# Li-Yuetao/ActiveSplat

Hardware: AMD Instinct MI355X
Metric: render+backward frames/sec at 640x480, N Gaussians (higher is better)
Workload: dtype f32; 1 GPU; BASELINE configs[2]'s render (the north star's target configuration): 2000000 Gaussians, SH degree 3, 640x480, forward (colour+radii+depth+opacity) + backward (all input gradients), frames strictly one after the other; gaussians=2000000, sh_degree=3, width=640, height=480, tile_instances_D=4842856, streams=1, parallelism=single GPU

## Files before the change

### activesplat_amd/csrc/gs_common.h

```cpp
#pragma once
#include <hip/hip_runtime.h>
#include <stdint.h>
#include <math.h>

#include <atomic>

#include "../../include/gsplat_hip.h"

namespace gs {

constexpr int kTile = GS_TILE;
constexpr int kBlock = 256;
constexpr int kWave = 64;
constexpr int kQuad = 8;
#ifndef GS_BIN_CHUNK
#define GS_BIN_CHUNK 2048
#endif
constexpr int kBinChunk = GS_BIN_CHUNK;
constexpr int kMaxLdsTiles = 8192;
constexpr int kSortChunk = 2048;
constexpr int kSortCapMax = 16384;

struct Cam {
    int W, H, gx, gy;
// ... 290 lines not shown
                                                    uint32_t row_mask = 0xffffffffu)
{
    const int K = KC > 0 ? KC : Krt;
    const int stride = sh_row_stride(K), total = nrows * K, total4 = total >> 2;
    const float* s = src + (size_t)row0 * K;
    const float4* s4 = reinterpret_cast<const float4*>(s);
    for (int q = lane; q < total4; q += kWave) {
        int e = q << 2, r = e / K, c = e - r * K;
        const int r_last = (e + 3) / K;
        if (!(((row_mask >> r) | (row_mask >> min(r_last, 31))) & 1u)) continue;
        const float4 v = load_stream(&s4[q]);
        const float vv[4] = {v.x, v.y, v.z, v.w};
#pragma unroll
        for (int t = 0; t < 4; t++) {
            slab[r * stride + c] = vv[t];
            if (++c == K) { c = 0; ++r; }
        }
    }
    for (int e = (total4 << 2) + lane; e < total; e += kWave) {
        const int r = e / K;
        if ((row_mask >> r) & 1u) slab[r * stride + (e - r * K)] = s[e];
    }
}
__device__ __forceinline__ void sh48_half_load(float4 (&v)[6], const float* __restrict__ src, int row0, int lane)
{
    const float4* s4 = reinterpret_cast<const float4*>(src + (size_t)row0 * 48);
#pragma unroll
    for (int j = 0; j < 6; j++) v[j] = load_stream(&s4[lane + kWave * j]);
}
constexpr int kShPad4 = 52;
__device__ __forceinline__ void sh48_half_to_lds4(float* slab, const float4 (&v)[6], int lane)
{
#pragma unroll
    for (int j = 0; j < 6; j++) {
        const int q = lane + kWave * j, r = q / 12, c = q - 12 * r;
        *reinterpret_cast<float4*>(slab + r * kShPad4 + 4 * c) = v[j];
    }
}
__device__ __forceinline__ void sh48_rows_to_lds4(float* slab, const float* __restrict__ src, int row0, int nrows, int lane, uint32_t row_mask = 0xffffffffu)
{
    const float4* s4 = reinterpret_cast<const float4*>(src + (size_t)row0 * 48);
    for (int q = lane; q < nrows * 12; q += kWave) {
        const int r = q / 12, c = q - 12 * r;
        if ((row_mask >> r) & 1u) *reinterpret_cast<float4*>(slab + r * kShPad4 + 4 * c) = load_stream(&s4[q]);
    }
}
template <int KC = 0>
__device__ __forceinline__ void sh_wave_rows_from_lds(const float* slab, float* __restrict__ dst, int row0, int nrows, int Krt, int lane)
{
    const int K = KC > 0 ? KC : Krt;
    const int stride = sh_row_stride(K), total = nrows * K, total4 = total >> 2;
    float* d = dst + (size_t)row0 * K;
    float4* d4 = reinterpret_cast<float4*>(d);
    for (int q = lane; q < total4; q += kWave) {
        int e = q << 2, r = e / K, c = e - r * K;
        float vv[4];
#pragma unroll
        for (int t = 0; t < 4; t++) {
            vv[t] = slab[r * stride + c];
            if (++c == K) { c = 0; ++r; }
        }
        store_stream(&d4[q], make_float4(vv[0], vv[1], vv[2], vv[3]));
    }
    for (int e = (total4 << 2) + lane; e < total; e += kWave) {
        const int r = e / K;
        d[e] = slab[r * stride + (e - r * K)];
    }
// ... 16 lines not shown
            by[5] = c21 * z; bz[5] = c21 * y;
            bx[6] = c22 * (-2.f * x); by[6] = c22 * (-2.f * y); bz[6] = c22 * (4.f * z);
            bx[7] = c23 * z; bz[7] = c23 * x;
            bx[8] = c24 * (2.f * x); by[8] = c24 * (-2.f * y);
            if (deg > 2) {
                const float c30 = -0.5900435899266435f, c31 = 2.890611442640554f, c32 = -0.4570457994644658f,
                            c33 = 0.3731763325901154f, c34 = -0.4570457994644658f, c35 = 1.445305721320277f,
                            c36 = -0.5900435899266435f;
                b[9] = c30 * y * (3.f * xx - yy); b[10] = c31 * x * y * z; b[11] = c32 * y * (4.f * zz - xx - yy);
                b[12] = c33 * z * (2.f * zz - 3.f * xx - 3.f * yy); b[13] = c34 * x * (4.f * zz - xx - yy);
                b[14] = c35 * z * (xx - yy); b[15] = c36 * x * (xx - 3.f * yy);
                bx[9] = c30 * (6.f * x * y); by[9] = c30 * (3.f * xx - 3.f * yy);
                bx[10] = c31 * y * z; by[10] = c31 * x * z; bz[10] = c31 * x * y;
                bx[11] = c32 * (-2.f * x * y); by[11] = c32 * (4.f * zz - xx - 3.f * yy); bz[11] = c32 * (8.f * y * z);
                bx[12] = c33 * (-6.f * x * z); by[12] = c33 * (-6.f * y * z); bz[12] = c33 * (6.f * zz - 3.f * xx - 3.f * yy);
                bx[13] = c34 * (4.f * zz - 3.f * xx - yy); by[13] = c34 * (-2.f * x * y); bz[13] = c34 * (8.f * x * z);
                bx[14] = c35 * (2.f * x * z); by[14] = c35 * (-2.f * y * z); bz[14] = c35 * (xx - yy);
                bx[15] = c36 * (3.f * xx - 3.f * yy); by[15] = c36 * (-6.f * x * y);
            }
        }
    }
}


#define GS_SHJ(k, gx, gy, gz)                                                                                                  \
    do {                                                                                                                        \
        const float c0_ = sh[3 * (k)], c1_ = sh[3 * (k) + 1], c2_ = sh[3 * (k) + 2];                                            \
        const float gx_ = (gx), gy_ = (gy), gz_ = (gz);                                                                         \
        J[0] = fmaf(c0_, gx_, J[0]); J[1] = fmaf(c0_, gy_, J[1]); J[2] = fmaf(c0_, gz_, J[2]);                                  \
        J[3] = fmaf(c1_, gx_, J[3]); J[4] = fmaf(c1_, gy_, J[4]); J[5] = fmaf(c1_, gz_, J[5]);                                  \
        J[6] = fmaf(c2_, gx_, J[6]); J[7] = fmaf(c2_, gy_, J[7]); J[8] = fmaf(c2_, gz_, J[8]);                                  \
    } while (0)
__device__ __forceinline__ void sh_direction_jacobian(int deg, float x, float y, float z, const float* sh, float (&J)[9])
{
#pragma unroll
    for (int q = 0; q < 9; q++) J[q] = 0.0f;
    if (deg < 1) return;
    const float C1 = 0.4886025119029199f;
    GS_SHJ(1, 0.f, -C1, 0.f); GS_SHJ(2, 0.f, 0.f, C1); GS_SHJ(3, -C1, 0.f, 0.f);
    if (deg < 2) return;
    const float c20 = 1.0925484305920792f, c21 = -1.0925484305920792f, c22 = 0.31539156525252005f, c23 = -1.0925484305920792f,
                c24 = 0.5462742152960396f;
    GS_SHJ(4, c20 * y, c20 * x, 0.f);
    GS_SHJ(5, 0.f, c21 * z, c21 * y);
    GS_SHJ(6, c22 * (-2.f * x), c22 * (-2.f * y), c22 * (4.f * z));
    GS_SHJ(7, c23 * z, 0.f, c23 * x);
// ... 35 lines not shown
{
    const double bc1 = 1.0 - pow(beta1, (double)step), bc2 = 1.0 - pow(beta2, (double)step);
    AdamCoef c;
    c.one_m_b1 = (float)(1.0 - beta1); c.b2 = (float)beta2; c.one_m_b2 = (float)(1.0 - beta2);
    c.step_size = (float)(lr / bc1); c.inv_bc2s = (float)(1.0 / sqrt(bc2)); c.eps = (float)eps;
    return c;
}

#define GS_SHC(j, k)                                                                                                           \
    do {                                                                                                                        \
        acc[0] = fmaf(b[k], f[3 * (j)], acc[0]); acc[1] = fmaf(b[k], f[3 * (j) + 1], acc[1]); acc[2] = fmaf(b[k], f[3 * (j) + 2], acc[2]);    \
    } while (0)
#define GS_SHJ4(j, gx, gy, gz)                                                                                                 \
    do {                                                                                                                        \
        const float c0_ = f[3 * (j)], c1_ = f[3 * (j) + 1], c2_ = f[3 * (j) + 2];                                               \
        const float gx_ = (gx), gy_ = (gy), gz_ = (gz);                                                                         \
        J[0] = fmaf(c0_, gx_, J[0]); J[1] = fmaf(c0_, gy_, J[1]); J[2] = fmaf(c0_, gz_, J[2]);                                  \
        J[3] = fmaf(c1_, gx_, J[3]); J[4] = fmaf(c1_, gy_, J[4]); J[5] = fmaf(c1_, gz_, J[5]);                                  \
        J[6] = fmaf(c2_, gx_, J[6]); J[7] = fmaf(c2_, gy_, J[7]); J[8] = fmaf(c2_, gz_, J[8]);                                  \
    } while (0)
#define GS_SHLOAD(g)                                                                                                           \
    const float4 q0_##g = row4[3 * (g)], q1_##g = row4[3 * (g) + 1], q2_##g = row4[3 * (g) + 2];                              \
    const float f[12] = {q0_##g.x, q0_##g.y, q0_##g.z, q0_##g.w, q1_##g.x, q1_##g.y, q1_##g.z, q1_##g.w, q2_##g.x, q2_##g.y, q2_##g.z, q2_##g.w}
__device__ __forceinline__ void sh48_color_and_jacobian(int deg, float x, float y, float z, const float (&b)[16], const float* row, bool want_j,
                                                        float (&acc)[3], float (&J)[9])
{
    const float4* row4 = reinterpret_cast<const float4*>(row);
#pragma unroll
    for (int q = 0; q < 9; q++) J[q] = 0.0f;
    acc[0] = acc[1] = acc[2] = 0.0f;
    const float C1 = 0.4886025119029199f;
    const float c20 = 1.0925484305920792f, c21 = -1.0925484305920792f, c22 = 0.31539156525252005f, c23 = -1.0925484305920792f,
                c24 = 0.5462742152960396f;
    const float c30 = -0.5900435899266435f, c31 = 2.890611442640554f, c32 = -0.4570457994644658f, c33 = 0.3731763325901154f,
                c34 = -0.4570457994644658f, c35 = 1.445305721320277f, c36 = -0.5900435899266435f;
    const float xx = x * x, yy = y * y, zz = z * z;
    {
        GS_SHLOAD(0);
        GS_SHC(0, 0);
        if (deg < 1) return;
        GS_SHC(1, 1); GS_SHC(2, 2); GS_SHC(3, 3);
        if (want_j) { GS_SHJ4(1, 0.f, -C1, 0.f); GS_SHJ4(2, 0.f, 0.f, C1); GS_SHJ4(3, -C1, 0.f, 0.f); }
    }
    if (deg < 2) return;
    {
        GS_SHLOAD(1);
        GS_SHC(0, 4); GS_SHC(1, 5); GS_SHC(2, 6); GS_SHC(3, 7);
        if (want_j) {
            GS_SHJ4(0, c20 * y, c20 * x, 0.f);
            GS_SHJ4(1, 0.f, c21 * z, c21 * y);
            GS_SHJ4(2, c22 * (-2.f * x), c22 * (-2.f * y), c22 * (4.f * z));
            GS_SHJ4(3, c23 * z, 0.f, c23 * x);
        }
    }
    {
        GS_SHLOAD(2);
        GS_SHC(0, 8);
        if (want_j) GS_SHJ4(0, c24 * (2.f * x), c24 * (-2.f * y), 0.f);
        if (deg >= 3) {
            GS_SHC(1, 9); GS_SHC(2, 10); GS_SHC(3, 11);
            if (want_j) {
                GS_SHJ4(1, c30 * (6.f * x * y), c30 * (3.f * xx - 3.f * yy), 0.f);
                GS_SHJ4(2, c31 * y * z, c31 * x * z, c31 * x * y);
                GS_SHJ4(3, c32 * (-2.f * x * y), c32 * (4.f * zz - xx - 3.f * yy), c32 * (8.f * y * z));
            }
        }
    }
    if (deg < 3) return;
    {
        GS_SHLOAD(3);
        GS_SHC(0, 12); GS_SHC(1, 13); GS_SHC(2, 14); GS_SHC(3, 15);
        if (want_j) {
            GS_SHJ4(0, c33 * (-6.f * x * z), c33 * (-6.f * y * z), c33 * (6.f * zz - 3.f * xx - 3.f * yy));
            GS_SHJ4(1, c34 * (4.f * zz - 3.f * xx - yy), c34 * (-2.f * x * y), c34 * (8.f * x * z));
            GS_SHJ4(2, c35 * (2.f * x * z), c35 * (-2.f * y * z), c35 * (xx - yy));
            GS_SHJ4(3, c36 * (3.f * xx - 3.f * yy), c36 * (-6.f * x * y), 0.f);
        }
    }
}
#undef GS_SHC
#undef GS_SHJ4
#undef GS_SHLOAD

constexpr int kShJacFloats = 10;
__device__ __forceinline__ void store_sh_jac(float2* base, size_t i, const float (&J)[9], uint32_t clamp_bits)
{
    float2* o = base + i * (kShJacFloats / 2);
    o[0] = make_float2(J[0], J[1]); o[1] = make_float2(J[2], J[3]); o[2] = make_float2(J[4], J[5]); o[3] = make_float2(J[6], J[7]);
    o[4] = make_float2(J[8], __uint_as_float(clamp_bits));
}
__device__ __forceinline__ void load_sh_jac(const float2* base, size_t i, float (&J)[9], uint32_t& clamp_bits)
{
    const float2* o = base + i * (kShJacFloats / 2);
    const float2 a = o[0], b = o[1], c = o[2], d = o[3], e = o[4];
    J[0] = a.x; J[1] = a.y; J[2] = b.x; J[3] = b.y; J[4] = c.x; J[5] = c.y; J[6] = d.x; J[7] = d.y; J[8] = e.x;
    clamp_bits = __float_as_uint(e.y);
}

hipError_t launch_preprocess_forward(const Cam& cam, int P, const float* means3D, const float* shs,
// ... 148 lines not shown
```

### activesplat_amd/csrc/preprocess.hip

```cpp
#include "gs_common.h"
#include <type_traits>

#pragma clang fp contract(off)

namespace gs {

__device__ __forceinline__ int clamp_tile(float v, int hi)
{
    v = fminf(fmaxf(v, -1048576.0f), 1048576.0f);
    int i = (int)v;
    return min(hi, max(0, i));
}

__device__ __forceinline__ void sh_basis(int deg, float x, float y, float z, float* b)
{
    b[0] = 0.28209479177387814f;
    if (deg > 0) {
        b[1] = -0.4886025119029199f * y; b[2] = 0.4886025119029199f * z; b[3] = -0.4886025119029199f * x;
        if (deg > 1) {
            const float xx = x * x, yy = y * y, zz = z * z, xy = x * y, yz = y * z, xz = x * z;
            b[4] = 1.0925484305920792f * xy;
            b[5] = -1.0925484305920792f * yz;
            b[6] = 0.31539156525252005f * (2.0f * zz - xx - yy);
            b[7] = -1.0925484305920792f * xz;
// ... 250 lines not shown
        __syncthreads();
    }
    int radius = 0;
    const uint32_t ntiles = project_gaussian<HAS_SH>(cam, P, view, i, io, tid, s_mean, s_scale, s_rot, s_cov, s_col, cov3Dp != nullptr, o_in,
                                                     sh_rgb, sh_clamp, radii, gp, ACT ? &radius : nullptr, in_band);
    if (ACT && i < P) {
        if (gp.vis_max) gp.vis_max[i] = fmaxf(gp.vis_max[i], (float)radius);
        if (gp.vis_seen) gp.vis_seen[i] = radius > 0 ? 1 : 0;
    }
    const uint32_t ws = wave_sum_u32(ntiles);
    if ((tid & 63) == 0) s_wsum[tid >> 6] = ws;
    __syncthreads();
    if (tid == 0) gp.block_sums[blockIdx.x] = s_wsum[0] + s_wsum[1] + s_wsum[2] + s_wsum[3];
}

template <bool ACT, class CamT = Cam>
__global__ __launch_bounds__(kBlock, 4) void preprocess_forward_sh48_kernel(
    typename CamArg<CamT>::type cam, int P, const float* __restrict__ means3D, const float* __restrict__ shs, const float* __restrict__ opac,
    const float* __restrict__ scales, const float* __restrict__ rots, const float* __restrict__ cov3Dp, int32_t* __restrict__ radii, GeomPtrs gp)
{
    load_device_pose(cam);
    __shared__ __attribute__((aligned(16))) float s_mean[kBlock * 3];
    __shared__ __attribute__((aligned(16))) float s_geo[kBlock * 7];
    __shared__ __attribute__((aligned(16))) float s_sh[(kBlock / kWave) * kShHalf * kShPad4];
    __shared__ uint32_t s_wsum[kBlock / kWave];
    float* const s_scale = s_geo;
    float* const s_rot = s_geo + kBlock * 3;
    float* const s_cov = s_geo;

    const int tid = threadIdx.x, lane = tid & 63, wave = tid >> 6;
    const int vbase = blockIdx.x * kBlock;
    const int view = cam.V > 1 ? (int)blockIdx.x / cam.nbv : 0;
    const int base = (cam.V > 1 ? (int)blockIdx.x - view * cam.nbv : (int)blockIdx.x) * kBlock;
    const int nrows = max(0, min(kBlock, P - base));
    if (vbase + tid < cam.gx * cam.gy) gp.tile_total[vbase + tid] = 0u;
    const int i = base + tid, io = vbase + tid;
    const int row_w = base + wave * kWave;
    const bool full = row_w + kWave <= P;
    float4 va[6];
    if (full) sh48_half_load(va, shs, row_w, lane);
    float o_in = i < P ? opac[i] : 0.0f;
    stage_rows<3>(s_mean, means3D, base, nrows, tid);
    if (cov3Dp) stage_rows<6>(s_cov, cov3Dp, base, nrows, tid);
    else {
        if (ACT && cam.act_iso) stage_rows<1>(s_scale, scales, base, nrows, tid); else stage_rows<3>(s_scale, scales, base, nrows, tid);
        stage_rows<4>(s_rot, rots, base, nrows, tid);
    }
    __syncthreads();
    if (ACT) o_in = activate_staged_rows(cam, tid, tid < nrows, s_mean, s_scale, s_rot, o_in);

    float sh_rgb[3] = {0.f, 0.f, 0.f};
    uint32_t sh_clamp = 0;
    float* slab = s_sh + wave * kShHalf * kShPad4;
    for (int h = 0; h < kWave / kShHalf; h++) {
        const int row0 = row_w + h * kShHalf;
        if (row0 >= P) break;
        __builtin_amdgcn_wave_barrier();
        if (full) {
            sh48_half_to_lds4(slab, va, lane);
            if (h == 0) sh48_half_load(va, shs, row_w + kShHalf, lane);
        } else {
            sh48_rows_to_lds4(slab, shs, row0, min(kShHalf, P - row0), lane);
        }
        __builtin_amdgcn_wave_barrier();
        if ((lane >> 5) == h && i < P) {
            const float* cp = cam.campos + 3 * view;
            const float dx = s_mean[tid * 3] - cp[0], dy = s_mean[tid * 3 + 1] - cp[1], dz = s_mean[tid * 3 + 2] - cp[2];
            const float inv = 1.0f / sqrtf((dx * dx + dy * dy) + dz * dz);
            float b[16];
            sh_basis(cam.sh_degree, dx * inv, dy * inv, dz * inv, b);
            float acc[3], J[9];
            sh48_color_and_jacobian(cam.sh_degree, dx * inv, dy * inv, dz * inv, b, slab + (lane & 31) * kShPad4, gp.sh_jac != nullptr, acc, J);
            acc[0] += 0.5f; acc[1] += 0.5f; acc[2] += 0.5f;
            sh_clamp = (acc[0] < 0.f ? 1u : 0u) | (acc[1] < 0.f ? 0x100u : 0u) | (acc[2] < 0.f ? 0x10000u : 0u);
            if (gp.sh_jac) store_sh_jac(gp.sh_jac, (size_t)io, J, sh_clamp);
                sh_rgb[0] = acc[0] < 0.f ? 0.f : acc[0]; sh_rgb[1] = acc[1] < 0.f ? 0.f : acc[1]; sh_rgb[2] = acc[2] < 0.f ? 0.f : acc[2];
        }
    }
    int radius = 0;
    const uint32_t ntiles = project_gaussian<true>(cam, P, view, i, io, tid, s_mean, s_scale, s_rot, s_cov, nullptr, cov3Dp != nullptr, o_in,
                                                   sh_rgb, sh_clamp, radii, gp, ACT ? &radius : nullptr);
    if (ACT && i < P) {
        if (gp.vis_max) gp.vis_max[i] = fmaxf(gp.vis_max[i], (float)radius);
        if (gp.vis_seen) gp.vis_seen[i] = radius > 0 ? 1 : 0;
    }
    const uint32_t ws = wave_sum_u32(ntiles);
    if (lane == 0) s_wsum[wave] = ws;
    __syncthreads();
    if (tid == 0) gp.block_sums[blockIdx.x] = s_wsum[0] + s_wsum[1] + s_wsum[2] + s_wsum[3];
}

__global__ __launch_bounds__(1024) void scan_block_sums_kernel(uint32_t* __restrict__ block_sums, int n, uint32_t* __restrict__ d_total)
{
    __shared__ uint32_t s_w[16];
    __shared__ uint32_t s_carry;
    const int tid = threadIdx.x, lane = tid & 63, wave = tid >> 6;
    if (tid == 0) s_carry = 0;
    __syncthreads();
    for (int base = 0; base < n; base += 1024) {
// ... 84 lines not shown
```

### activesplat_amd/csrc/preprocess_bwd.hip

```cpp
#include "gs_common.h"

namespace gs {

#ifndef GS_PBWD_RAW_SH_WGS
#define GS_PBWD_RAW_SH_WGS 4
#endif
template <bool NOALIAS> struct ParamPtr { typedef const float* __restrict__ type; };
template <> struct ParamPtr<false> { typedef const float* type; };

template <int SH, bool ACT = false, bool ADAM = false, int POSE = 0, class CamT = Cam>
__global__ __launch_bounds__(kBlock, (ACT && SH == 3) ? GS_PBWD_RAW_SH_WGS : 4) void preprocess_backward_kernel(
    typename CamArg<CamT>::type cam, int P, typename ParamPtr<!ADAM>::type means3D, typename ParamPtr<!ADAM>::type shs,
    typename ParamPtr<!ADAM>::type scales, typename ParamPtr<!ADAM>::type rots, const float* __restrict__ cov3Dp,
    const int32_t* __restrict__ radii, const uint32_t* __restrict__ clamped, const float2* __restrict__ sh_jac,
    const float* __restrict__ grad2d, float* __restrict__ dmeans2D, float* __restrict__ dmeans3D, float* __restrict__ dopac,
    float* __restrict__ dcolors, float* __restrict__ dshs, float* __restrict__ dscales,
    float* __restrict__ drots, float* __restrict__ dcov3D, typename ParamPtr<!ADAM>::type logit, FusedAdam ad, float* __restrict__ pose_rows)
{
    static_assert(POSE == 0 || (ACT && !ADAM && SH != 1), "the pose gradient is a raw-parameter mode without the optimiser step");
    load_device_pose(cam);
    float pacc[kPoseAcc];
    for (int k = 0; k < kPoseAcc; k++) pacc[k] = 0.f;
#define GS_PBWD_LEAVE do { if (POSE != 0) goto pose_reduce; return; } while (0)
    {
    constexpr bool HAS_SH = SH != 0;
    constexpr bool SLAB = SH == 1 || SH == 3;
    __shared__ __attribute__((aligned(16))) float s_sh[SLAB ? (kBlock / kWave) * kShHalf * kShPad : 1];
    const int tid = threadIdx.x;
    const int i = blockIdx.x * kBlock + tid;
    const bool in_range = i < P;
    if (ADAM && chain_failed(ad.fail)) {
        if (in_range) { dmeans2D[3 * i] = 0.f; dmeans2D[3 * i + 1] = 0.f; dmeans2D[3 * i + 2] = 0.f; }
        return;
    }
    if (!HAS_SH && !in_range) GS_PBWD_LEAVE;
    const int ic = in_range ? i : P - 1;
    const bool live = in_range && radii[ic] > 0;
    const float4* gr4 = reinterpret_cast<const float4*>(grad2d + (size_t)ic * kGradStride);
    const bool gate = ACT && !ADAM && !SLAB && cam.act_accumulate;
    float4 ga, gb, gc;
    if (gate) {
        if (!__any(live)) {
            if (in_range) { dmeans2D[3 * i] = 0.f; dmeans2D[3 * i + 1] = 0.f; dmeans2D[3 * i + 2] = 0.f; }
            GS_PBWD_LEAVE;
        }
        const float4 z4 = make_float4(0.f, 0.f, 0.f, 0.f);
        ga = z4; gb = z4; gc = z4;
        if (live) { ga = gr4[0]; gb = gr4[1]; gc = gr4[2]; }
    } else {
        ga = gr4[0]; gb = gr4[1]; gc = gr4[2];
    }
    float dmean[3] = {0.f, 0.f, 0.f};
    float o_m2d[3] = {0.f, 0.f, 0.f}, o_sc[3] = {0.f, 0.f, 0.f}, o_rot[4] = {0.f, 0.f, 0.f, 0.f};
    float o_cov[6] = {0.f, 0.f, 0.f, 0.f, 0.f, 0.f};
    float px = means3D[3 * ic], py = means3D[3 * ic + 1], pz = means3D[3 * ic + 2];
    float actR[3][3];
    if (ACT) {
        quat_to_rot(cam.act_q, actR);
        const float wx = px, wy = py, wz = pz;
        px = actR[0][0] * wx + actR[0][1] * wy + actR[0][2] * wz + cam.act_t[0];
        py = actR[1][0] * wx + actR[1][1] * wy + actR[1][2] * wz + cam.act_t[1];
        pz = actR[2][0] * wx + actR[2][1] * wy + actR[2][2] * wz + cam.act_t[2];
    }
    const float drgb[3] = {gb.z, gb.w, gc.x};
    uint32_t cl_in = 0u;
    float jac[9] = {0.f, 0.f, 0.f, 0.f, 0.f, 0.f, 0.f, 0.f, 0.f};
    if (HAS_SH && sh_jac) load_sh_jac(sh_jac, (size_t)ic, jac, cl_in);
    else if (HAS_SH) cl_in = clamped[ic];
    float sc_in[3] = {0.f, 0.f, 0.f};
    float4 rq_in = make_float4(0.f, 0.f, 0.f, 0.f), rq_raw = rq_in;
    float lg_in = 0.f;
    float cov_in[6] = {0.f, 0.f, 0.f, 0.f, 0.f, 0.f};
    if (cov3Dp) {
        for (int c = 0; c < 6; c++) cov_in[c] = cov3Dp[(size_t)ic * 6 + c];
    } else if (ACT) {
        if (cam.act_iso) { sc_in[0] = sc_in[1] = sc_in[2] = __expf(scales[ic]); }
        else { sc_in[0] = __expf(scales[3 * ic]); sc_in[1] = __expf(scales[3 * ic + 1]); sc_in[2] = __expf(scales[3 * ic + 2]); }
        rq_raw = reinterpret_cast<const float4*>(rots)[ic];
        lg_in = logit[ic];
        if (!live) {
            sc_in[0] = sc_in[1] = sc_in[2] = 0.f;
            rq_raw = make_float4(1.f, 0.f, 0.f, 0.f);
            lg_in = 0.f;
        }
        const float qr[4] = {rq_raw.x, rq_raw.y, rq_raw.z, rq_raw.w};
        float qa[4];
        activate_rotation(cam.act_q, cam.act_iso, qr, qa);
        rq_in = make_float4(qa[0], qa[1], qa[2], qa[3]);
    } else {
        sc_in[0] = scales[3 * ic]; sc_in[1] = scales[3 * ic + 1]; sc_in[2] = scales[3 * ic + 2];
        rq_in = reinterpret_cast<const float4*>(rots)[ic];
    }
    if (SLAB) {
        constexpr int KC = SH == 3 ? 48 : 0;
        const int deg = cam.sh_degree, nb = (deg + 1) * (deg + 1), M = KC ? 16 : cam.sh_coeffs, K = M * 3;
        const int stride = sh_row_stride(K);
        const int lane = tid & 63, wave = tid >> 6;
        float* slab = s_sh + wave * kShHalf * kShPad;
        for (int h = 0; h < kWave / kShHalf; h++) {
            const int row0 = blockIdx.x * kBlock + wave * kWave + h * kShHalf;
            if (row0 >= P) break;
            const int nrows = min(kShHalf, P - row0);
            __builtin_amdgcn_wave_barrier();
            const uint32_t live_rows = (uint32_t)(__ballot(live) >> (h * kShHalf));
            if (!sh_jac) sh_wave_rows_to_lds<KC>(slab, shs, row0, nrows, K, lane, live_rows);
            __builtin_amdgcn_wave_barrier();
            if ((lane >> 5) == h && in_range) {
                float* dsh = slab + (lane & 31) * stride;
                if (live) {
                    const float dx = px - cam.campos[0], dy = py - cam.campos[1], dz = pz - cam.campos[2];
                    const float inv = 1.0f / sqrtf(dx * dx + dy * dy + dz * dz);
                    const float ux = dx * inv, uy = dy * inv, uz = dz * inv;
                    float b[16], bx[16], by[16], bz[16];
                    sh_basis_and_grad(deg, ux, uy, uz, b, bx, by, bz);
                    const uint32_t cl = cl_in;
                    float du[3] = {0.f, 0.f, 0.f};
                    if (ADAM || sh_jac) {
                        const float jr[3][3] = {{jac[0], jac[1], jac[2]}, {jac[3], jac[4], jac[5]}, {jac[6], jac[7], jac[8]}};
                        for (int ch = 0; ch < 3; ch++) {
                            const float g = ((cl >> (8 * ch)) & 1u) ? 0.f : drgb[ch];
                            du[0] += g * jr[ch][0]; du[1] += g * jr[ch][1]; du[2] += g * jr[ch][2];
#pragma unroll
                            for (int k = 0; k < 16; k++)
                                if (k < M) dsh[3 * k + ch] = k < nb ? g * b[k] : 0.f;
                        }
                    } else {
                        for (int ch = 0; ch < 3; ch++) {
                            const float g = ((cl >> (8 * ch)) & 1u) ? 0.f : drgb[ch];
#pragma unroll
                            for (int k = 0; k < 16; k++) {
                                if (k < nb) {
                                    const float coef = dsh[3 * k + ch];
                                    dsh[3 * k + ch] = g * b[k];
                                    du[0] += g * coef * bx[k]; du[1] += g * coef * by[k]; du[2] += g * coef * bz[k];
                                } else if (k < M) {
                                    dsh[3 * k + ch] = 0.f;
                                }
                            }
                        }
                    }
                    const float dot = ux * du[0] + uy * du[1] + uz * du[2];
                    dmean[0] += (du[0] - ux * dot) * inv; dmean[1] += (du[1] - uy * dot) * inv; dmean[2] += (du[2] - uz * dot) * inv;
                } else {
                    for (int k = 0; k < K; k++) dsh[k] = 0.f;
                }
            }
            __builtin_amdgcn_wave_barrier();
            if (ADAM) {
                float4* p4 = reinterpret_cast<float4*>(ad.p[4] + (size_t)row0 * K);
                float4* m4 = reinterpret_cast<float4*>(ad.m[4] + (size_t)row0 * K);
                float4* v4 = reinterpret_cast<float4*>(ad.v[4] + (size_t)row0 * K);
                const int total4 = (nrows * K) >> 2;
                for (int q4 = lane; q4 < total4; q4 += kWave) {
                    float4 pp = load_stream(&p4[q4]), mm = load_stream(&m4[q4]), vv = load_stream(&v4[q4]);
                    const int e = q4 << 2, rr = e / K, cc = e - rr * K;
                    const float* gs_ = slab + rr * stride + cc;
                    adam_elem(pp.x, gs_[0], mm.x, vv.x, ad.c[4]); adam_elem(pp.y, gs_[1], mm.y, vv.y, ad.c[4]);
                    adam_elem(pp.z, gs_[2], mm.z, vv.z, ad.c[4]); adam_elem(pp.w, gs_[3], mm.w, vv.w, ad.c[4]);
                    store_stream(&p4[q4], pp); store_stream(&m4[q4], mm); store_stream(&v4[q4], vv);
                }
            } else if (POSE != 2) {
                sh_wave_rows_from_lds<KC>(slab, dshs, row0, nrows, K, lane);
            }
        }
        if (!in_range) GS_PBWD_LEAVE;
    }
    if (live) {
        const float* m = cam.view;
        const float* q = cam.proj;
        const float tx = m[0] * px + m[4] * py + m[8] * pz + m[12];
        const float ty = m[1] * px + m[5] * py + m[9] * pz + m[13];
        const float tz = m[2] * px + m[6] * py + m[10] * pz + m[14];
        const float limx = 1.3f * cam.tanfovx, limy = 1.3f * cam.tanfovy;
        const float txtz = tx / tz, tytz = ty / tz;
        const bool okx = !(txtz < -limx || txtz > limx), oky = !(tytz < -limy || tytz > limy);
        const float cx_ = fminf(limx, fmaxf(-limx, txtz)) * tz, cy_ = fminf(limy, fmaxf(-limy, tytz)) * tz;
        const float itz = 1.0f / tz, itz2 = itz * itz, itz3 = itz2 * itz;
        const float J00 = cam.fx * itz, J02 = -(cam.fx * cx_) * itz2, J11 = cam.fy * itz, J12 = -(cam.fy * cy_) * itz2;
        const float W0[3] = {m[0], m[4], m[8]}, W1[3] = {m[1], m[5], m[9]}, W2[3] = {m[2], m[6], m[10]};
        float T0[3], T1[3];
        for (int c = 0; c < 3; c++) { T0[c] = J00 * W0[c] + J02 * W2[c]; T1[c] = J11 * W1[c] + J12 * W2[c]; }
        float ST0[3], ST1[3];
        float Rm[3][3], s3[3] = {0.f, 0.f, 0.f};
        float r = 0.f, x = 0.f, y = 0.f, z = 0.f;
// ... 167 lines not shown
    if (dcolors) for (int c = 0; c < 3; c++) dcolors[3 * i + c] = live ? drgb[c] : 0.f;
    if (dscales) for (int c = 0; c < 3; c++) dscales[3 * i + c] = o_sc[c];
    if (drots) reinterpret_cast<float4*>(drots)[i] = make_float4(o_rot[0], o_rot[1], o_rot[2], o_rot[3]);
    if (dcov3D) for (int c = 0; c < 6; c++) dcov3D[6 * i + c] = o_cov[c];
    }
#undef GS_PBWD_LEAVE
    return;
pose_reduce:
    if (POSE != 0) pose_grad_block_row(pacc, pose_rows + (size_t)blockIdx.x * kPoseAcc);
}

hipError_t launch_preprocess_backward(const Cam& cam, int P, const float* means3D, const float* shs,
                                      const float* scales, const float* rots, const float* cov3Dp,
                                      const int32_t* radii, const uint32_t* clamped, const float2* sh_jac, const float* grad2d,
                                      float* dmeans2D, float* dmeans3D, float* dopac, float* dcolors, float* dshs,
                                      float* dscales, float* drots, float* dcov3D, const float* logit, const FusedAdam* adam, hipStream_t st,
                                      int pose_mode, float* pose_rows)
{
    const int nb = (P + kBlock - 1) / kBlock;
    const bool pose_only = pose_mode == 2;
    if (cam.act && (cov3Dp || !logit || !scales || !rots || (!adam && !pose_only && (!dscales || !drots)) || (shs && cam.sh_coeffs != 16))) return hipErrorInvalidValue;
    if (adam && (!cam.act || cam.act_accumulate)) return hipErrorInvalidValue;
    if (pose_mode && (!cam.act || adam || !pose_rows || pose_mode > 2)) return hipErrorInvalidValue;
    const FusedAdam ad = adam ? *adam : FusedAdam{};
#define GS_PBWD(...) hipLaunchKernelGGL((preprocess_backward_kernel<__VA_ARGS__>), dim3(nb), dim3(kBlock), 0, st, cam, P, means3D, shs, scales, rots, \
                                        cov3Dp, radii, clamped, sh_jac, grad2d, dmeans2D, dmeans3D, dopac, dcolors, dshs, dscales, drots, dcov3D, logit, ad, \
                                        pose_rows)
    if (nb > 0 && pose_mode) {
        if (shs) { if (pose_only) GS_PBWD(3, true, false, 2, Cam); else GS_PBWD(3, true, false, 1, Cam); }
        else { if (pose_only) GS_PBWD(0, true, false, 2, Cam); else GS_PBWD(0, true, false, 1, Cam); }
    }
    else if (nb > 0 && shs && cam.sh_coeffs == 16) { if (adam) GS_PBWD(3, true, true); else if (cam.act) GS_PBWD(3, true); else GS_PBWD(3, false); }
    else if (nb > 0 && shs) GS_PBWD(1, false);
    else if (nb > 0) { if (adam) GS_PBWD(0, true, true); else if (cam.act) GS_PBWD(0, true); else GS_PBWD(0, false); }
#undef GS_PBWD
    return hipGetLastError();
}

hipError_t launch_preprocess_backward_pose_dev(const CamDP& cam, int P, const float* means3D, const float* shs, const float* scales,
                                               const float* rots, const int32_t* radii, const uint32_t* clamped, const float2* sh_jac,
                                               const float* grad2d, float* dmeans2D, const float* logit, float* pose_rows, hipStream_t st)
{
    const int nb = (P + kBlock - 1) / kBlock;
    if (!cam.act || !logit || !scales || !rots || !pose_rows || (shs && cam.sh_coeffs != 16)) return hipErrorInvalidValue;
    const FusedAdam ad{};
#define GS_PBWD_DEV(SH_) hipLaunchKernelGGL((preprocess_backward_kernel<SH_, true, false, 2, CamDP>), dim3(nb), dim3(kBlock), 0, st, cam, P, means3D, \
                                            shs, scales, rots, nullptr, radii, clamped, sh_jac, grad2d, dmeans2D, nullptr, nullptr, nullptr, \
                                            nullptr, nullptr, nullptr, nullptr, logit, ad, pose_rows)
    if (nb > 0 && shs) GS_PBWD_DEV(3);
    else if (nb > 0) GS_PBWD_DEV(0);
#undef GS_PBWD_DEV
    return hipGetLastError();
}

}
```

Measured before the change: 1491 frames/s.

## Stage SH coefficients in column halves and skip backward SH re-read with saved Jacobian

The forward preprocess now stages each wave's 64 SH rows in two coefficient halves (24 floats per row, padded to 28) in LDS, so every lane handles its own Gaussian in each pass instead of half the wave idling over 32-row halves. The second half is skipped when the SH degree is below 2. In the backward, when a saved SH Jacobian is available (or Adam is fused), a new path writes dSH straight from the basis times the colour gradient in two halves. It no longer loads the SH coefficients or computes basis gradients, and takes the direction gradient from the saved Jacobian. This cuts global reads and ALU in the backward, at the cost of a new template parameter and a requirement that Adam always has sh_jac.

```diff
diff --git a/activesplat_amd/csrc/gs_common.h b/activesplat_amd/csrc/gs_common.h
--- a/activesplat_amd/csrc/gs_common.h
+++ b/activesplat_amd/csrc/gs_common.h
@@ -336,27 +336,47 @@
         if ((row_mask >> r) & 1u) slab[r * stride + (e - r * K)] = s[e];
     }
 }
-__device__ __forceinline__ void sh48_half_load(float4 (&v)[6], const float* __restrict__ src, int row0, int lane)
-{
-    const float4* s4 = reinterpret_cast<const float4*>(src + (size_t)row0 * 48);
-#pragma unroll
-    for (int j = 0; j < 6; j++) v[j] = load_stream(&s4[lane + kWave * j]);
-}
-constexpr int kShPad4 = 52;
-__device__ __forceinline__ void sh48_half_to_lds4(float* slab, const float4 (&v)[6], int lane)
-{
+constexpr int kShCoefHalf = 24;
+constexpr int kShPadC = 28;
+__device__ __forceinline__ float4 sh48_load_piece(const float4* p, bool stream)
+{
+    return stream ? load_stream(p) : *p;
+}
+__device__ __forceinline__ void sh48_chalf_load(float4 (&v)[6], const float* __restrict__ src, int row0, int half, int lane, bool stream)
+{
+    const float4* s4 = reinterpret_cast<const float4*>(src + (size_t)row0 * 48) + 6 * half;
 #pragma unroll
     for (int j = 0; j < 6; j++) {
-        const int q = lane + kWave * j, r = q / 12, c = q - 12 * r;
-        *reinterpret_cast<float4*>(slab + r * kShPad4 + 4 * c) = v[j];
-    }
-}
-__device__ __forceinline__ void sh48_rows_to_lds4(float* slab, const float* __restrict__ src, int row0, int nrows, int lane, uint32_t row_mask = 0xffffffffu)
-{
-    const float4* s4 = reinterpret_cast<const float4*>(src + (size_t)row0 * 48);
-    for (int q = lane; q < nrows * 12; q += kWave) {
-        const int r = q / 12, c = q - 12 * r;
-        if ((row_mask >> r) & 1u) *reinterpret_cast<float4*>(slab + r * kShPad4 + 4 * c) = load_stream(&s4[q]);
+        const int q = lane + kWave * j, r = q / 6, c = q - 6 * r;
+        v[j] = sh48_load_piece(&s4[12 * r + c], stream);
+    }
+}
+__device__ __forceinline__ void sh48_chalf_to_lds(float* slab, const float4 (&v)[6], int lane)
+{
+#pragma unroll
+    for (int j = 0; j < 6; j++) {
+        const int q = lane + kWave * j, r = q / 6, c = q - 6 * r;
+        *reinterpret_cast<float4*>(slab + r * kShPadC + 4 * c) = v[j];
+    }
+}
+__device__ __forceinline__ void sh48_chalf_rows_to_lds(float* slab, const float* __restrict__ src, int row0, int nrows, int half, int lane, bool stream)
+{
+    const float4* s4 = reinterpret_cast<const float4*>(src + (size_t)row0 * 48) + 6 * half;
+    for (int q = lane; q < nrows * 6; q += kWave) {
+        const int r = q / 6, c = q - 6 * r;
+        *reinterpret_cast<float4*>(slab + r * kShPadC + 4 * c) = sh48_load_piece(&s4[12 * r + c], stream);
+    }
+}
+__device__ __forceinline__ void sh48_store_piece(float4* p, const float4& x, bool stream)
+{
+    if (stream) store_stream(p, x); else *p = x;
+}
+__device__ __forceinline__ void sh48_chalf_rows_from_lds(const float* slab, float* __restrict__ dst, int row0, int nrows, int half, int lane, bool stream)
+{
+    float4* d4 = reinterpret_cast<float4*>(dst + (size_t)row0 * 48) + 6 * half;
+    for (int q = lane; q < nrows * 6; q += kWave) {
+        const int r = q / 6, c = q - 6 * r;
+        sh48_store_piece(&d4[12 * r + c], *reinterpret_cast<const float4*>(slab + r * kShPadC + 4 * c), stream);
     }
 }
 template <int KC = 0>
@@ -419,6 +439,29 @@
     }
 }
 
+__device__ __forceinline__ void sh_basis16(int deg, float x, float y, float z, float* b)
+{
+    for (int k = 0; k < 16; k++) b[k] = 0.f;
+    const float C1 = 0.4886025119029199f;
+    b[0] = 0.28209479177387814f;
+    if (deg > 0) {
+        b[1] = -C1 * y; b[2] = C1 * z; b[3] = -C1 * x;
+        if (deg > 1) {
+            const float c20 = 1.0925484305920792f, c21 = -1.0925484305920792f, c22 = 0.31539156525252005f,
+                        c23 = -1.0925484305920792f, c24 = 0.5462742152960396f;
+            const float xx = x * x, yy = y * y, zz = z * z;
+            b[4] = c20 * x * y; b[5] = c21 * y * z; b[6] = c22 * (2.f * zz - xx - yy); b[7] = c23 * x * z; b[8] = c24 * (xx - yy);
+            if (deg > 2) {
+                const float c30 = -0.5900435899266435f, c31 = 2.890611442640554f, c32 = -0.4570457994644658f,
+                            c33 = 0.3731763325901154f, c34 = -0.4570457994644658f, c35 = 1.445305721320277f,
+                            c36 = -0.5900435899266435f;
+                b[9] = c30 * y * (3.f * xx - yy); b[10] = c31 * x * y * z; b[11] = c32 * y * (4.f * zz - xx - yy);
+                b[12] = c33 * z * (2.f * zz - 3.f * xx - 3.f * yy); b[13] = c34 * x * (4.f * zz - xx - yy);
+                b[14] = c35 * z * (xx - yy); b[15] = c36 * x * (xx - 3.f * yy);
+            }
+        }
+    }
+}
 
 #define GS_SHJ(k, gx, gy, gz)                                                                                                  \
     do {                                                                                                                        \
@@ -500,59 +543,64 @@
 #define GS_SHLOAD(g)                                                                                                           \
     const float4 q0_##g = row4[3 * (g)], q1_##g = row4[3 * (g) + 1], q2_##g = row4[3 * (g) + 2];                              \
     const float f[12] = {q0_##g.x, q0_##g.y, q0_##g.z, q0_##g.w, q1_##g.x, q1_##g.y, q1_##g.z, q1_##g.w, q2_##g.x, q2_##g.y, q2_##g.z, q2_##g.w}
-__device__ __forceinline__ void sh48_color_and_jacobian(int deg, float x, float y, float z, const float (&b)[16], const float* row, bool want_j,
-                                                        float (&acc)[3], float (&J)[9])
-{
-    const float4* row4 = reinterpret_cast<const float4*>(row);
-#pragma unroll
-    for (int q = 0; q < 9; q++) J[q] = 0.0f;
-    acc[0] = acc[1] = acc[2] = 0.0f;
+template <int HALF>
+__device__ __forceinline__ void sh48_chalf_color_and_jacobian(int deg, float x, float y, float z, const float (&b)[16], const float* half_row,
+                                                              bool want_j, float (&acc)[3], float (&J)[9])
+{
+    const float4* row4 = reinterpret_cast<const float4*>(half_row);
     const float C1 = 0.4886025119029199f;
     const float c20 = 1.0925484305920792f, c21 = -1.0925484305920792f, c22 = 0.31539156525252005f, c23 = -1.0925484305920792f,
                 c24 = 0.5462742152960396f;
     const float c30 = -0.5900435899266435f, c31 = 2.890611442640554f, c32 = -0.4570457994644658f, c33 = 0.3731763325901154f,
                 c34 = -0.4570457994644658f, c35 = 1.445305721320277f, c36 = -0.5900435899266435f;
     const float xx = x * x, yy = y * y, zz = z * z;
-    {
-        GS_SHLOAD(0);
-        GS_SHC(0, 0);
-        if (deg < 1) return;
-        GS_SHC(1, 1); GS_SHC(2, 2); GS_SHC(3, 3);
-        if (want_j) { GS_SHJ4(1, 0.f, -C1, 0.f); GS_SHJ4(2, 0.f, 0.f, C1); GS_SHJ4(3, -C1, 0.f, 0.f); }
-    }
-    if (deg < 2) return;
-    {
-        GS_SHLOAD(1);
-        GS_SHC(0, 4); GS_SHC(1, 5); GS_SHC(2, 6); GS_SHC(3, 7);
-        if (want_j) {
-            GS_SHJ4(0, c20 * y, c20 * x, 0.f);
-            GS_SHJ4(1, 0.f, c21 * z, c21 * y);
-            GS_SHJ4(2, c22 * (-2.f * x), c22 * (-2.f * y), c22 * (4.f * z));
-            GS_SHJ4(3, c23 * z, 0.f, c23 * x);
+    if (HALF == 0) {
+#pragma unroll
+        for (int q = 0; q < 9; q++) J[q] = 0.0f;
+        acc[0] = acc[1] = acc[2] = 0.0f;
+        {
+            GS_SHLOAD(0);
+            GS_SHC(0, 0);
+            if (deg < 1) return;
+            GS_SHC(1, 1); GS_SHC(2, 2); GS_SHC(3, 3);
+            if (want_j) { GS_SHJ4(1, 0.f, -C1, 0.f); GS_SHJ4(2, 0.f, 0.f, C1); GS_SHJ4(3, -C1, 0.f, 0.f); }
         }
-    }
-    {
-        GS_SHLOAD(2);
-        GS_SHC(0, 8);
-        if (want_j) GS_SHJ4(0, c24 * (2.f * x), c24 * (-2.f * y), 0.f);
-        if (deg >= 3) {
-            GS_SHC(1, 9); GS_SHC(2, 10); GS_SHC(3, 11);
+        if (deg < 2) return;
+        {
+            GS_SHLOAD(1);
+            GS_SHC(0, 4); GS_SHC(1, 5); GS_SHC(2, 6); GS_SHC(3, 7);
             if (want_j) {
-                GS_SHJ4(1, c30 * (6.f * x * y), c30 * (3.f * xx - 3.f * yy), 0.f);
-                GS_SHJ4(2, c31 * y * z, c31 * x * z, c31 * x * y);
-                GS_SHJ4(3, c32 * (-2.f * x * y), c32 * (4.f * zz - xx - 3.f * yy), c32 * (8.f * y * z));
+                GS_SHJ4(0, c20 * y, c20 * x, 0.f);
+                GS_SHJ4(1, 0.f, c21 * z, c21 * y);
+                GS_SHJ4(2, c22 * (-2.f * x), c22 * (-2.f * y), c22 * (4.f * z));
+                GS_SHJ4(3, c23 * z, 0.f, c23 * x);
             }
         }
-    }
-    if (deg < 3) return;
-    {
-        GS_SHLOAD(3);
-        GS_SHC(0, 12); GS_SHC(1, 13); GS_SHC(2, 14); GS_SHC(3, 15);
-        if (want_j) {
-            GS_SHJ4(0, c33 * (-6.f * x * z), c33 * (-6.f * y * z), c33 * (6.f * zz - 3.f * xx - 3.f * yy));
-            GS_SHJ4(1, c34 * (4.f * zz - 3.f * xx - yy), c34 * (-2.f * x * y), c34 * (8.f * x * z));
-            GS_SHJ4(2, c35 * (2.f * x * z), c35 * (-2.f * y * z), c35 * (xx - yy));
-            GS_SHJ4(3, c36 * (3.f * xx - 3.f * yy), c36 * (-6.f * x * y), 0.f);
+    } else {
+        if (deg < 2) return;
+        {
+            GS_SHLOAD(0);
+            GS_SHC(0, 8);
+            if (want_j) GS_SHJ4(0, c24 * (2.f * x), c24 * (-2.f * y), 0.f);
+            if (deg >= 3) {
+                GS_SHC(1, 9); GS_SHC(2, 10); GS_SHC(3, 11);
+                if (want_j) {
+                    GS_SHJ4(1, c30 * (6.f * x * y), c30 * (3.f * xx - 3.f * yy), 0.f);
+                    GS_SHJ4(2, c31 * y * z, c31 * x * z, c31 * x * y);
+                    GS_SHJ4(3, c32 * (-2.f * x * y), c32 * (4.f * zz - xx - 3.f * yy), c32 * (8.f * y * z));
+                }
+            }
+        }
+        if (deg < 3) return;
+        {
+            GS_SHLOAD(1);
+            GS_SHC(0, 12); GS_SHC(1, 13); GS_SHC(2, 14); GS_SHC(3, 15);
+            if (want_j) {
+                GS_SHJ4(0, c33 * (-6.f * x * z), c33 * (-6.f * y * z), c33 * (6.f * zz - 3.f * xx - 3.f * yy));
+                GS_SHJ4(1, c34 * (4.f * zz - 3.f * xx - yy), c34 * (-2.f * x * y), c34 * (8.f * x * z));
+                GS_SHJ4(2, c35 * (2.f * x * z), c35 * (-2.f * y * z), c35 * (xx - yy));
+                GS_SHJ4(3, c36 * (3.f * xx - 3.f * yy), c36 * (-6.f * x * y), 0.f);
+            }
         }
     }
 }
diff --git a/activesplat_amd/csrc/preprocess.hip b/activesplat_amd/csrc/preprocess.hip
--- a/activesplat_amd/csrc/preprocess.hip
+++ b/activesplat_amd/csrc/preprocess.hip
@@ -296,7 +296,7 @@
     load_device_pose(cam);
     __shared__ __attribute__((aligned(16))) float s_mean[kBlock * 3];
     __shared__ __attribute__((aligned(16))) float s_geo[kBlock * 7];
-    __shared__ __attribute__((aligned(16))) float s_sh[(kBlock / kWave) * kShHalf * kShPad4];
+    __shared__ __attribute__((aligned(16))) float s_sh[kBlock * kShPadC];
     __shared__ uint32_t s_wsum[kBlock / kWave];
     float* const s_scale = s_geo;
     float* const s_rot = s_geo + kBlock * 3;
@@ -312,7 +312,7 @@
     const int row_w = base + wave * kWave;
     const bool full = row_w + kWave <= P;
     float4 va[6];
-    if (full) sh48_half_load(va, shs, row_w, lane);
+    if (full) sh48_chalf_load(va, shs, row_w, 0, lane, false);
     float o_in = i < P ? opac[i] : 0.0f;
     stage_rows<3>(s_mean, means3D, base, nrows, tid);
     if (cov3Dp) stage_rows<6>(s_cov, cov3Dp, base, nrows, tid);
@@ -325,30 +325,45 @@
 
     float sh_rgb[3] = {0.f, 0.f, 0.f};
     uint32_t sh_clamp = 0;
-    float* slab = s_sh + wave * kShHalf * kShPad4;
-    for (int h = 0; h < kWave / kShHalf; h++) {
-        const int row0 = row_w + h * kShHalf;
-        if (row0 >= P) break;
+    if (row_w < P) {
+        float* slab = s_sh + wave * kWave * kShPadC;
+        const float* half_row = slab + lane * kShPadC;
+        const int deg = cam.sh_degree;
+        const bool second = deg >= 2;
+        const int wrows = P - row_w;
+        if (full) {
+            sh48_chalf_to_lds(slab, va, lane);
+            if (second) sh48_chalf_load(va, shs, row_w, 1, lane, true);
+        } else {
+            sh48_chalf_rows_to_lds(slab, shs, row_w, wrows, 0, lane, false);
+        }
         __builtin_amdgcn_wave_barrier();
-        if (full) {
-            sh48_half_to_lds4(slab, va, lane);
-            if (h == 0) sh48_half_load(va, shs, row_w + kShHalf, lane);
-        } else {
-            sh48_rows_to_lds4(slab, shs, row0, min(kShHalf, P - row0), lane);
-        }
-        __builtin_amdgcn_wave_barrier();
-        if ((lane >> 5) == h && i < P) {
+        float ux = 0.f, uy = 0.f, uz = 0.f, acc[3] = {0.f, 0.f, 0.f}, J[9];
+        if (i < P) {
             const float* cp = cam.campos + 3 * view;
             const float dx = s_mean[tid * 3] - cp[0], dy = s_mean[tid * 3 + 1] - cp[1], dz = s_mean[tid * 3 + 2] - cp[2];
             const float inv = 1.0f / sqrtf((dx * dx + dy * dy) + dz * dz);
+            ux = dx * inv; uy = dy * inv; uz = dz * inv;
             float b[16];
-            sh_basis(cam.sh_degree, dx * inv, dy * inv, dz * inv, b);
-            float acc[3], J[9];
-            sh48_color_and_jacobian(cam.sh_degree, dx * inv, dy * inv, dz * inv, b, slab + (lane & 31) * kShPad4, gp.sh_jac != nullptr, acc, J);
+            sh_basis(deg, ux, uy, uz, b);
+            sh48_chalf_color_and_jacobian<0>(deg, ux, uy, uz, b, half_row, gp.sh_jac != nullptr, acc, J);
+        }
+        if (second) {
+            __builtin_amdgcn_wave_barrier();
+            if (full) sh48_chalf_to_lds(slab, va, lane);
+            else sh48_chalf_rows_to_lds(slab, shs, row_w, wrows, 1, lane, true);
+            __builtin_amdgcn_wave_barrier();
+            if (i < P) {
+                float b[16];
+                sh_basis(deg, ux, uy, uz, b);
+                sh48_chalf_color_and_jacobian<1>(deg, ux, uy, uz, b, half_row, gp.sh_jac != nullptr, acc, J);
+            }
+        }
+        if (i < P) {
             acc[0] += 0.5f; acc[1] += 0.5f; acc[2] += 0.5f;
             sh_clamp = (acc[0] < 0.f ? 1u : 0u) | (acc[1] < 0.f ? 0x100u : 0u) | (acc[2] < 0.f ? 0x10000u : 0u);
             if (gp.sh_jac) store_sh_jac(gp.sh_jac, (size_t)io, J, sh_clamp);
-                sh_rgb[0] = acc[0] < 0.f ? 0.f : acc[0]; sh_rgb[1] = acc[1] < 0.f ? 0.f : acc[1]; sh_rgb[2] = acc[2] < 0.f ? 0.f : acc[2];
+            sh_rgb[0] = acc[0] < 0.f ? 0.f : acc[0]; sh_rgb[1] = acc[1] < 0.f ? 0.f : acc[1]; sh_rgb[2] = acc[2] < 0.f ? 0.f : acc[2];
         }
     }
     int radius = 0;
diff --git a/activesplat_amd/csrc/preprocess_bwd.hip b/activesplat_amd/csrc/preprocess_bwd.hip
--- a/activesplat_amd/csrc/preprocess_bwd.hip
+++ b/activesplat_amd/csrc/preprocess_bwd.hip
@@ -8,7 +8,7 @@
 template <bool NOALIAS> struct ParamPtr { typedef const float* __restrict__ type; };
 template <> struct ParamPtr<false> { typedef const float* type; };
 
-template <int SH, bool ACT = false, bool ADAM = false, int POSE = 0, class CamT = Cam>
+template <int SH, bool ACT = false, bool ADAM = false, int POSE = 0, class CamT = Cam, bool JAC = false>
 __global__ __launch_bounds__(kBlock, (ACT && SH == 3) ? GS_PBWD_RAW_SH_WGS : 4) void preprocess_backward_kernel(
     typename CamArg<CamT>::type cam, int P, typename ParamPtr<!ADAM>::type means3D, typename ParamPtr<!ADAM>::type shs,
     typename ParamPtr<!ADAM>::type scales, typename ParamPtr<!ADAM>::type rots, const float* __restrict__ cov3Dp,
@@ -25,7 +25,9 @@
     {
     constexpr bool HAS_SH = SH != 0;
     constexpr bool SLAB = SH == 1 || SH == 3;
-    __shared__ __attribute__((aligned(16))) float s_sh[SLAB ? (kBlock / kWave) * kShHalf * kShPad : 1];
+    constexpr bool SAVED = HAS_SH && (JAC || ADAM);
+    constexpr bool CPASS = SAVED && SH == 3;
+    __shared__ __attribute__((aligned(16))) float s_sh[CPASS ? kBlock * kShPadC : SLAB ? (kBlock / kWave) * kShHalf * kShPad : 1];
     const int tid = threadIdx.x;
     const int i = blockIdx.x * kBlock + tid;
     const bool in_range = i < P;
@@ -65,7 +67,7 @@
     const float drgb[3] = {gb.z, gb.w, gc.x};
     uint32_t cl_in = 0u;
     float jac[9] = {0.f, 0.f, 0.f, 0.f, 0.f, 0.f, 0.f, 0.f, 0.f};
-    if (HAS_SH && sh_jac) load_sh_jac(sh_jac, (size_t)ic, jac, cl_in);
+    if (HAS_SH && (SAVED || sh_jac)) load_sh_jac(sh_jac, (size_t)ic, jac, cl_in);
     else if (HAS_SH) cl_in = clamped[ic];
     float sc_in[3] = {0.f, 0.f, 0.f};
     float4 rq_in = make_float4(0.f, 0.f, 0.f, 0.f), rq_raw = rq_in;
@@ -91,7 +93,62 @@
         sc_in[0] = scales[3 * ic]; sc_in[1] = scales[3 * ic + 1]; sc_in[2] = scales[3 * ic + 2];
         rq_in = reinterpret_cast<const float4*>(rots)[ic];
     }
-    if (SLAB) {
+    if (CPASS) {
+        const int deg = cam.sh_degree, nb = (deg + 1) * (deg + 1);
+        const int lane = tid & 63, wave = tid >> 6;
+        const int row_w = blockIdx.x * kBlock + wave * kWave;
+        if (row_w < P) {
+            const int wrows = min(kWave, P - row_w);
+            float* slab = s_sh + wave * kWave * kShPadC;
+            float4* dsh4 = reinterpret_cast<float4*>(slab + lane * kShPadC);
+            float b[16], g[3] = {0.f, 0.f, 0.f};
+            for (int k = 0; k < 16; k++) b[k] = 0.f;
+            if (live) {
+                const float dx = px - cam.campos[0], dy = py - cam.campos[1], dz = pz - cam.campos[2];
+                const float inv = 1.0f / sqrtf(dx * dx + dy * dy + dz * dz);
+                const float ux = dx * inv, uy = dy * inv, uz = dz * inv;
+                sh_basis16(deg, ux, uy, uz, b);
+                float du[3] = {0.f, 0.f, 0.f};
+                const float jr[3][3] = {{jac[0], jac[1], jac[2]}, {jac[3], jac[4], jac[5]}, {jac[6], jac[7], jac[8]}};
+                for (int ch = 0; ch < 3; ch++) {
+                    if ((cl_in >> (8 * ch)) & 1u) continue;
+                    g[ch] = drgb[ch];
+                    du[0] += g[ch] * jr[ch][0]; du[1] += g[ch] * jr[ch][1]; du[2] += g[ch] * jr[ch][2];
+                }
+                const float dot = ux * du[0] + uy * du[1] + uz * du[2];
+                dmean[0] += (du[0] - ux * dot) * inv; dmean[1] += (du[1] - uy * dot) * inv; dmean[2] += (du[2] - uz * dot) * inv;
+            }
+#pragma unroll
+            for (int half = 0; half < 2; half++) {
+                if (half) __builtin_amdgcn_wave_barrier();
+                if (in_range) {
+                    float v[kShCoefHalf];
+#pragma unroll
+                    for (int k = 0; k < 8; k++)
+                        for (int ch = 0; ch < 3; ch++) v[3 * k + ch] = (live && 8 * half + k < nb) ? g[ch] * b[8 * half + k] : 0.f;
+#pragma unroll
+                    for (int c = 0; c < 6; c++) dsh4[c] = make_float4(v[4 * c], v[4 * c + 1], v[4 * c + 2], v[4 * c + 3]);
+                }
+                __builtin_amdgcn_wave_barrier();
+                if (ADAM) {
+                    float4* p4 = reinterpret_cast<float4*>(ad.p[4] + (size_t)row_w * 48) + 6 * half;
+                    float4* m4 = reinterpret_cast<float4*>(ad.m[4] + (size_t)row_w * 48) + 6 * half;
+                    float4* v4 = reinterpret_cast<float4*>(ad.v[4] + (size_t)row_w * 48) + 6 * half;
+                    for (int q = lane; q < wrows * 6; q += kWave) {
+                        const int rr = q / 6, cc = q - 6 * rr, e = 12 * rr + cc;
+                        float4 pp = sh48_load_piece(&p4[e], half != 0), mm = sh48_load_piece(&m4[e], half != 0), vv = sh48_load_piece(&v4[e], half != 0);
+                        const float4 gs_ = *reinterpret_cast<const float4*>(slab + rr * kShPadC + 4 * cc);
+                        adam_elem(pp.x, gs_.x, mm.x, vv.x, ad.c[4]); adam_elem(pp.y, gs_.y, mm.y, vv.y, ad.c[4]);
+                        adam_elem(pp.z, gs_.z, mm.z, vv.z, ad.c[4]); adam_elem(pp.w, gs_.w, mm.w, vv.w, ad.c[4]);
+                        sh48_store_piece(&p4[e], pp, half != 0); sh48_store_piece(&m4[e], mm, half != 0); sh48_store_piece(&v4[e], vv, half != 0);
+                    }
+                } else if (POSE != 2) {
+                    sh48_chalf_rows_from_lds(slab, dshs, row_w, wrows, half, lane, half != 0);
+                }
+            }
+        }
+        if (!in_range) GS_PBWD_LEAVE;
+    } else if (SLAB) {
         constexpr int KC = SH == 3 ? 48 : 0;
         const int deg = cam.sh_degree, nb = (deg + 1) * (deg + 1), M = KC ? 16 : cam.sh_coeffs, K = M * 3;
         const int stride = sh_row_stride(K);
@@ -115,7 +172,7 @@
                     sh_basis_and_grad(deg, ux, uy, uz, b, bx, by, bz);
                     const uint32_t cl = cl_in;
                     float du[3] = {0.f, 0.f, 0.f};
-                    if (ADAM || sh_jac) {
+                    if (sh_jac) {
                         const float jr[3][3] = {{jac[0], jac[1], jac[2]}, {jac[3], jac[4], jac[5]}, {jac[6], jac[7], jac[8]}};
                         for (int ch = 0; ch < 3; ch++) {
                             const float g = ((cl >> (8 * ch)) & 1u) ? 0.f : drgb[ch];
@@ -146,20 +203,7 @@
                 }
             }
             __builtin_amdgcn_wave_barrier();
-            if (ADAM) {
-                float4* p4 = reinterpret_cast<float4*>(ad.p[4] + (size_t)row0 * K);
-                float4* m4 = reinterpret_cast<float4*>(ad.m[4] + (size_t)row0 * K);
-                float4* v4 = reinterpret_cast<float4*>(ad.v[4] + (size_t)row0 * K);
-                const int total4 = (nrows * K) >> 2;
-                for (int q4 = lane; q4 < total4; q4 += kWave) {
-                    float4 pp = load_stream(&p4[q4]), mm = load_stream(&m4[q4]), vv = load_stream(&v4[q4]);
-                    const int e = q4 << 2, rr = e / K, cc = e - rr * K;
-                    const float* gs_ = slab + rr * stride + cc;
-                    adam_elem(pp.x, gs_[0], mm.x, vv.x, ad.c[4]); adam_elem(pp.y, gs_[1], mm.y, vv.y, ad.c[4]);
-                    adam_elem(pp.z, gs_[2], mm.z, vv.z, ad.c[4]); adam_elem(pp.w, gs_[3], mm.w, vv.w, ad.c[4]);
-                    store_stream(&p4[q4], pp); store_stream(&m4[q4], mm); store_stream(&v4[q4], vv);
-                }
-            } else if (POSE != 2) {
+            if (POSE != 2) {
                 sh_wave_rows_from_lds<KC>(slab, dshs, row0, nrows, K, lane);
             }
         }
@@ -373,17 +417,23 @@
     if (cam.act && (cov3Dp || !logit || !scales || !rots || (!adam && !pose_only && (!dscales || !drots)) || (shs && cam.sh_coeffs != 16))) return hipErrorInvalidValue;
     if (adam && (!cam.act || cam.act_accumulate)) return hipErrorInvalidValue;
     if (pose_mode && (!cam.act || adam || !pose_rows || pose_mode > 2)) return hipErrorInvalidValue;
+    if (adam && shs && !sh_jac) return hipErrorInvalidValue;
+    const bool jac = shs && sh_jac;
     const FusedAdam ad = adam ? *adam : FusedAdam{};
 #define GS_PBWD(...) hipLaunchKernelGGL((preprocess_backward_kernel<__VA_ARGS__>), dim3(nb), dim3(kBlock), 0, st, cam, P, means3D, shs, scales, rots, \
                                         cov3Dp, radii, clamped, sh_jac, grad2d, dmeans2D, dmeans3D, dopac, dcolors, dshs, dscales, drots, dcov3D, logit, ad, \
                                         pose_rows)
+#define GS_PBWD_J(...) do { if (jac) GS_PBWD(__VA_ARGS__, true); else GS_PBWD(__VA_ARGS__, false); } while (0)
     if (nb > 0 && pose_mode) {
-        if (shs) { if (pose_only) GS_PBWD(3, true, false, 2, Cam); else GS_PBWD(3, true, false, 1, Cam); }
-        else { if (pose_only) GS_PBWD(0, true, false, 2, Cam); else GS_PBWD(0, true, false, 1, Cam); }
-    }
-    else if (nb > 0 && shs && cam.sh_coeffs == 16) { if (adam) GS_PBWD(3, true, true); else if (cam.act) GS_PBWD(3, true); else GS_PBWD(3, false); }
+        if (shs) { if (pose_only) GS_PBWD_J(3, true, false, 2, Cam); else GS_PBWD_J(3, true, false, 1, Cam); }
+        else { if (pose_only) GS_PBWD(0, true, false, 2, Cam, false); else GS_PBWD(0, true, false, 1, Cam, false); }
+    }
+    else if (nb > 0 && shs && cam.sh_coeffs == 16) {
+        if (adam) GS_PBWD(3, true, true); else if (cam.act) GS_PBWD_J(3, true, false, 0, Cam); else GS_PBWD_J(3, false, false, 0, Cam);
+    }
     else if (nb > 0 && shs) GS_PBWD(1, false);
     else if (nb > 0) { if (adam) GS_PBWD(0, true, true); else if (cam.act) GS_PBWD(0, true); else GS_PBWD(0, false); }
+#undef GS_PBWD_J
 #undef GS_PBWD
     return hipGetLastError();
 }
@@ -395,11 +445,11 @@
     const int nb = (P + kBlock - 1) / kBlock;
     if (!cam.act || !logit || !scales || !rots || !pose_rows || (shs && cam.sh_coeffs != 16)) return hipErrorInvalidValue;
     const FusedAdam ad{};
-#define GS_PBWD_DEV(SH_) hipLaunchKernelGGL((preprocess_backward_kernel<SH_, true, false, 2, CamDP>), dim3(nb), dim3(kBlock), 0, st, cam, P, means3D, \
+#define GS_PBWD_DEV(SH_, JAC_) hipLaunchKernelGGL((preprocess_backward_kernel<SH_, true, false, 2, CamDP, JAC_>), dim3(nb), dim3(kBlock), 0, st, cam, P, means3D, \
                                             shs, scales, rots, nullptr, radii, clamped, sh_jac, grad2d, dmeans2D, nullptr, nullptr, nullptr, \
                                             nullptr, nullptr, nullptr, nullptr, logit, ad, pose_rows)
-    if (nb > 0 && shs) GS_PBWD_DEV(3);
-    else if (nb > 0) GS_PBWD_DEV(0);
+    if (nb > 0 && shs) { if (sh_jac) GS_PBWD_DEV(3, true); else GS_PBWD_DEV(3, false); }
+    else if (nb > 0) GS_PBWD_DEV(0, false);
 #undef GS_PBWD_DEV
     return hipGetLastError();
 }
```

Result: slower. 1385 frames/s (-7.1%).
